# Janspiry/Image-Super-Resolution-via-Iterative-Refinement

Hardware: NVIDIA H100
Metric: diffusion steps/sec (batch16, 16->128 SR3) (higher is better)
Workload: dtype bf16

## Files before the change

### image-super-resolution-via-iterative-refinement_b200/_native.py

```python
import ctypes
import os
from ctypes import POINTER, c_char_p, c_double, c_float, c_int, c_int64, c_uint64, c_void_p

import torch

_PKG = os.path.dirname(os.path.abspath(__file__))
LIB_PATH = os.path.join(_PKG, "lib", "libsr3_b200.so")
SR3_MAX_LEVELS = 8
_lib = None


class NativeLibraryError(RuntimeError):
    pass


class UNetConfigC(ctypes.Structure):
    _fields_ = [("in_channel", c_int), ("out_channel", c_int), ("inner_channel", c_int), ("norm_groups", c_int),
                ("n_mults", c_int), ("channel_mults", c_int * SR3_MAX_LEVELS), ("n_attn_res", c_int),
                ("attn_res", c_int * SR3_MAX_LEVELS), ("res_blocks", c_int), ("image_size", c_int), ("channels", c_int),
                ("conditional", c_int), ("precision", c_int)]


PRECISIONS = {"bf16": 0, "fp32": 1}


class GemmGeometryC(ctypes.Structure):
    _fields_ = [(n, c_int) for n in ("tall", "mh", "block_n", "h_box", "b_box", "ksplit", "stages", "ctas", "tiles", "res_smem")]


class TestConvArgsC(ctypes.Structure):
    _fields_ = [("x", c_void_p), ("w", c_void_p), ("bias", c_void_p), ("bias2", c_void_p), ("resid", c_void_p),
                ("x2", c_void_p), ("w2", c_void_p),
                ("y", c_void_p), ("y_bf16", c_void_p), ("stats", c_void_p)] + \
               [(n, c_int) for n in ("B", "H", "W", "Cin", "Cout", "Cin2", "ksize", "stride", "fold_up", "precise")]


class TestGroupNormArgsC(ctypes.Structure):
    _fields_ = [(n, c_void_p) for n in ("x0", "x1", "st0", "st1", "gamma", "beta", "drop_mask", "dA", "add", "a_bf16", "mr", "dst0", "dst0_b",
                                         "gsum0", "dst1", "dgamma", "dbeta")] + \
               [("drop_seed", c_uint64)] + [(n, c_int) for n in ("B", "HW", "C0", "C1", "groups", "silu", "drop", "add_ld", "acc0")] + \
               [("drop_layer", ctypes.c_uint), ("drop_p", c_float), ("gscale", c_float)]


class TestFilmArgsC(ctypes.Structure):
    _fields_ = [(n, c_void_p) for n in ("wf", "tau", "dfilm", "nl", "w1", "b1", "w2", "dwf", "dbf", "dcb", "dtau", "dw1", "db1", "dw2", "db2")] + \
               [(n, c_int) for n in ("F", "inner", "B")] + [("gscale", c_float)]


_SIGS = {
    "sr3_last_error": (c_char_p, []),
    "sr3_abi_version": (c_int, []),
    "sr3_engine_create": (c_int, [POINTER(UNetConfigC), c_int, c_int, POINTER(c_void_p)]),
    "sr3_engine_create_sized": (c_int, [POINTER(UNetConfigC), c_int, c_int, c_int, c_int, POINTER(c_void_p)]),
    "sr3_engine_create_train": (c_int, [POINTER(UNetConfigC), c_int, c_int, c_float, POINTER(c_void_p)]),
    "sr3_train_forward": (c_int, [c_void_p, c_void_p, c_void_p, c_void_p, c_void_p, c_int, c_uint64, POINTER(c_double), c_void_p]),
    "sr3_train_backward": (c_int, [c_void_p, c_float, POINTER(c_void_p), c_int, c_void_p]),
    "sr3_train_num_backward_blocks": (c_int, [c_void_p]),
    "sr3_train_backward_begin": (c_int, [c_void_p, c_float, POINTER(c_void_p), c_int]),
    "sr3_train_backward_block": (c_int, [c_void_p, c_int, c_void_p]),
    "sr3_train_backward_flush": (c_int, [c_void_p, c_void_p]),
# ... 634 lines not shown
```

### image-super-resolution-via-iterative-refinement_b200/csrc/engine.cu

```cuda
#include <cuda.h>
#include <cuda_runtime.h>

#include <cmath>
#include <cstdarg>
#include <cstdlib>
#include <cstring>
#include <functional>
#include <limits>
#include <map>
#include <memory>
#include <mutex>
#include <stdexcept>
#include <string>
#include <vector>

#include "../../include/sr3_b200.h"
#include "aux_kernels.cuh"
#include "attn_wgmma.cuh"
#include "step_megakernel.cuh"
#include "train_kernels.cuh"

using namespace sr3;
typedef __nv_bfloat16 bf16;

// ... 362 lines not shown
        if (!d.out_f32) p.out_map = p.res_map;
        if (!d.resid) p.res_map = p.out_map;
        p.epi_c4_is_z = (d.out_f32 ? zo : zr) ? 1 : 0;
    } else {
        p.out_map = p.b_map; p.res_map = p.b_map;
    }
    p.ksplit = 1;
    {
        const int tiles = d.tiles_w * d.tiles_h * d.tiles_b * d.n_tiles * d.nz;
        const int ks = d.ksplit_max;
        if (ks > 1 && !d.pingpong && d.mode == 0 && d.out_f32 && d.block_n >= 32 && d.n_valid % 32 == 0) {
            int want = num_sms() / tiles;
            if (want > ks) want = ks;
            if (want > p.num_k * d.passes / 2) want = p.num_k * d.passes / 2;
            const int units = d.mh * (d.block_n / 32) * 4;
            if (want > units) want = units;
            want = fit_split(want, tiles);
            if (want > 1) {
                p.ksplit = want;
                p.ws = static_cast<float*>(mem.alloc((size_t)tiles * want * d.mh * 128 * d.block_n * sizeof(float), false));
                p.counters = static_cast<unsigned int*>(mem.alloc((size_t)tiles * sizeof(unsigned int)));
            }
        }
    }
    const int total_tiles = d.tiles_w * d.tiles_h * d.tiles_b * d.n_tiles * d.nz * p.ksplit;
    int ctas = total_tiles < num_sms() ? total_tiles : num_sms();
    if (const char* e = getenv("SR3_MAX_CTAS")) { int v = atoi(e); if (v > 0 && v < ctas) ctas = v; }
    REQUIRE(p.ksplit == 1 || ctas == total_tiles, "split-K launch needs one CTA per (tile, split) pair: %d CTAs for %d (SR3_MAX_CTAS with a split tile)", ctas, total_tiles);
    const dim3 grid(ctas, 1, 1);
    const int bn = d.block_n;
    const int mh = d.mh;
    const bool res_smem = p.tma_epi && d.resid != nullptr && p.ksplit <= 1;
    p.stages = pick_stages(d.block_n, p.a_stage_bytes, p.b_taps, res_smem, p.num_k);
    const int smem = gemm_smem_bytes(bn, p.a_stage_bytes, p.b_taps, p.stages, res_smem, p.num_k);
    REQUIRE(smem <= SMEM_LIMIT, "gemm shared memory %d exceeds the limit", smem);
    init_gemm_attrs();
    REQUIRE((bn == 16 || bn == 32 || bn == 64 || bn == 128 || bn == 256) && (mh == 1 || (mh == 2 && bn <= 128 && bn != 32)), "unsupported tile %dx%d", 128 * mh, bn);
    const bool pp = d.pingpong != 0;
    REQUIRE(!pp || (gemm_pingpong_ok(bn, mh) && p.ksplit == 1 && d.mode == 0), "no ping-pong form of tile %dx%d (split %d)", 128 * mh, bn, p.ksplit);
    if (geo) {
        geo->tall = d.tall; geo->mh = mh; geo->block_n = bn; geo->h_box = d.h_box; geo->b_box = d.b_box;
        geo->ksplit = p.ksplit; geo->stages = p.stages; geo->ctas = ctas; geo->tiles = total_tiles / p.ksplit; geo->res_smem = res_smem ? 1 : 0;
    }
    if (schedule) *schedule = pp ? 1 : 0;
    std::shared_ptr<GemmParams> sp = std::make_shared<GemmParams>(p);
    if (g_gemm_registry) {
        GemmHandle h; h.p = sp; h.w_ptr = d.b_ptr; h.w_bytes = 2LL * d.b_rows * d.b_K; h.w_is_param = d.b_is_param; h.bn = bn; h.mh = mh;
        g_gemm_registry->push_back(h);
    }
    if (g_mega_registry) {
        MegaRec r; r.type = MOP_GEMM; r.variant = bn | (mh << 16) | (pp ? MEGA_VARIANT_PP : 0); r.gp = sp;
        g_mega_registry->push_back(std::move(r));
    }
    return [sp, grid, bn, mh, pp, smem](cudaStream_t st) {
        const GemmParams& p = *sp;
        if (pp) {
            if (mh == 2) launch_gemm_bn<64, 2, true>(p, grid, smem, st);
            else if (bn == 64) launch_gemm_bn<64, 1, true>(p, grid, smem, st);
            else launch_gemm_bn<128, 1, true>(p, grid, smem, st);
            return;
        }
        switch (bn) {
            case 16: if (mh == 2) launch_gemm_bn<16, 2>(p, grid, smem, st); else launch_gemm_bn<16, 1>(p, grid, smem, st); break;
            case 32: launch_gemm_bn<32, 1>(p, grid, smem, st); break;
            case 64: if (mh == 2) launch_gemm_bn<64, 2>(p, grid, smem, st); else launch_gemm_bn<64, 1>(p, grid, smem, st); break;
            case 128: if (mh == 2) launch_gemm_bn<128, 2>(p, grid, smem, st); else launch_gemm_bn<128, 1>(p, grid, smem, st); break;
            default: launch_gemm_bn<256, 1>(p, grid, smem, st); break;
        }
    };
}

bool attn_fusable(int Lt, int C) { return (Lt == 128 || Lt == 256) && C % 128 == 0 && C >= 128; }

Op make_attn_op(const bf16* qk, const bf16* vT, bf16* out, int nz, int Lt, int HW, int C) {
    REQUIRE(attn_fusable(Lt, C) && Lt % HW == 0, "attention shape Lt=%d HW=%d C=%d is not supported by the fused kernel", Lt, HW, C);
// ... 698 lines not shown
    }
    void f32_param_into(const std::string& name, std::vector<int64_t> shape, float* dst) {
        if (dry) return;
        add_param(name, shape);
        PackDesc d{}; d.type = 0; d.dst = dst; d.n = params.back().numel; add_pack(name, d);
    }
    void conv_weight_param(const std::string& name, bf16* dst, int Cout, int Cin, int k, int ktot, int k_off, int cin_pad) {
        if (dry) return;
        add_param(name, {Cout, Cin, k, k});
        PackDesc d{}; d.type = 1; d.dst = dst; d.Cout = Cout; d.Cin = Cin; d.k = k; d.ld = PW * ktot; d.k_off = k_off; d.tap_stride = cin_pad;
        d.lo_off = precise ? ktot : 0;
        add_pack(name, d);
    }
    bf16* new_weight(int rows, int ktot) {
        if (dry) return nullptr;
        const int rows_pad = ((rows + 127) / 128) * 128;
        return static_cast<bf16*>(mem.alloc((size_t)rows_pad * PW * ktot * sizeof(bf16)));
    }
    void set_precise(GemmDesc& d, int c0, int c1, int ktot) {
        if (precise) set_precise_fields(d, c0, c1, ktot);
    }
    void push(Op op, int kind = 4, double flops = 0, double bytes = 0) {
        if (dry) return;
        if (bwd_sink) { bwd_sink->push_back(std::move(op)); bwd_kinds.back().push_back(kind); return; }
        ops.push_back(std::move(op));
        op_info.push_back({kind, flops, bytes, sr3_gemm_geometry{}, -1, {0, 0, 0}});
    }
    void push_gemm(const GemmDesc& d) {
        const double M = (double)d.OW * d.OH * d.OB * (d.nz > 1 && d.a_zstep == 0 ? d.nz : 1);
        const double K = 64.0 * d.slabs.size() * (d.passes > 1 ? d.passes : 1);
        const double N = d.n_valid;
        double bytes = N * K * 2;
        if (d.out_f32) bytes += M * N * 4;
        if (d.out_bf16) bytes += M * N * 2;
        if (d.resid) bytes += M * N * 4;
        double a_elems = 0;
        for (int i = 0; i < d.n_a; ++i) a_elems += (double)d.a[i].C * d.a[i].W * d.a[i].P * d.a[i].H * d.a[i].Bn;
        bytes += a_elems * 2;
        sr3_gemm_geometry geo{};
        int schedule = 0;
        push(make_gemm_op(d, mem, &geo, &schedule), 0, 2.0 * M * N * K, bytes);
        if (!dry && !bwd_sink) {
            OpInfo& info = op_info.back();
            info.geo = geo; info.schedule = schedule;
            info.out_hwc[0] = d.OH * (d.z_phase ? 2 : 1); info.out_hwc[1] = d.OW * (d.z_phase ? 2 : 1); info.out_hwc[2] = d.n_valid;
        }
    }

    float* last_mr = nullptr;
    void add_prep(const Act& s0, const Act* s1, const float* gamma, const float* beta, int groups, bool silu, bf16* out_a, bf16* out_raw, const DropSpec* drop = nullptr) {
        if (dry) return;
        PrepParams p = gn_op(s0.p, s0.stats, s0.C, s1 ? s1->p : nullptr, s1 ? s1->stats : nullptr, s1 ? s1->C : 0, gamma, beta, groups, s0.H * s0.W, silu);
        p.drop = drop;
        if (train) { last_mr = static_cast<float*>(mem.alloc((size_t)Bp * groups * 2 * sizeof(float))); p.save_mr = last_mr; }
        p.out_a = out_a; p.out_raw = out_raw; p.precise = precise ? 1 : 0;
        const int C = p.C0 + p.C1;
        const int vpp = C / 4;
        const RowLaunch L = prep_launch(C, groups, p.HW, B);
        p.pix_per_block = L.ppb;
        {
            PrepParams m = p;
            const int nth = GEMM_THREADS;
            const int kp = vpp > nth ? 1 : nth / vpp;
            int ipi = (4 * num_sms() + B / 2) / B; if (ipi < 1) ipi = 1;
            int mp = (p.HW + ipi - 1) / ipi;
            mp = ((mp + kp - 1) / kp) * kp;
            if (mp > p.HW) mp = p.HW;
// ... 1524 lines not shown
```

### image-super-resolution-via-iterative-refinement_b200/csrc/gemm_wgmma.cuh

```cuda
#pragma once
#include <cuda.h>
#include <type_traits>
#include "ptx.cuh"

namespace sr3 {

struct OutSpec {
    long long sZ, sB, sH, sW, off;
};

struct StepCtl {
    int t_cur;
    int t_next;
    int nl_from_table;
    int out_mode;
    int use_noise_buf;
    int write_mean;
    int clip;
    int update_state;
    unsigned long long seed;
    unsigned long long sample_offset;
};

struct PostParams {
// ... 8 lines not shown
    int in_C, in_coff;
    int in_lo_off;
};

struct StageTap {
    int a_chan;
    int dw, dh, p;
    int b_col;
    int a_off;
};
struct StageDesc {
    int ntaps;
    int a_multi;
    int a_sel;
    int pad0;
    StageTap tap[3];
    int pad1, pad2;
};

struct GemmParams {
    CUtensorMap a_map[2];
    CUtensorMap b_map;
    CUtensorMap out_map;
    CUtensorMap res_map;
    const StageDesc* ktab;
    int num_k;
    int a_stage_bytes;
    int a_box_bytes;
    int a_half_off;
    int b_taps;
    int tiles_w, tiles_h, tiles_b;
    int n_tiles, nz;
    int tma_epi;
    int epi_c4_is_z;
    int ksplit;
    float* ws;
    unsigned int* counters;
    const void* pf_ptr;
    long long pf_bytes;
    int w_box, h_box, b_box;
    int w_shift, h_shift;
    int a_zstep, b_zrows;
    int stages;
    int mode;
    int OW, OH, OB, n_valid;
    float scale;
    const float* bias;
    const float* bias2;
    int bias2_stride;
    const float* resid;
    OutSpec rs;
    float* out_f32;
    OutSpec os;
    __nv_bfloat16* out_bf16;
    OutSpec hs;
    __nv_bfloat16* out_t;
    int t_col0, t_rows, t_ld, t_per;
    double* stats;
    int stats_C, stats_coff;
    const StepCtl* ctl;
    PostParams post;
    int z_phase;
    long long z_off_hi, z_off_lo;
    int passes, lo_b_col, lo_a_chan[2];
    long long lo_out_off, lo_t_off;
    int t_fixed;
};

constexpr int GEMM_THREADS = 288;
constexpr int GEMM_EPI_WARPS = 8;
constexpr int GEMM_PRODUCER_WARP = 8;
constexpr int GEMM_MAX_STAGES = 8;
__host__ __device__ constexpr int gemm_epi_warp_bytes(bool resid) { return resid ? 12288 : 4096; }
__host__ __device__ constexpr int gemm_epi_bytes(bool resid) { return GEMM_EPI_WARPS * gemm_epi_warp_bytes(resid); }
constexpr int GEMM_MAX_K = 160;
constexpr int GEMM_HDR_BYTES = 2048;
constexpr int HDR_SCALARS = 512;
constexpr int HDR_PARAMS = 768;
constexpr int HDR_NUM_BARS = 64;
__host__ __device__ constexpr bool gemm_single_wg(int block_n, int mh) { return mh == 1 && block_n <= 32; }
__host__ __device__ constexpr bool gemm_pingpong_ok(int block_n, int mh) { return (mh == 2 && block_n == 64) || (mh == 1 && (block_n == 64 || block_n == 128)); }
constexpr int GEMM_ORDER_BAR = 2;
__host__ __device__ constexpr int gemm_stage_readers(int block_n, int mh, bool pp) { return (pp || gemm_single_wg(block_n, mh)) ? 1 : 2; }
__host__ __device__ constexpr int gemm_aux_bytes(int num_k) {
    return GEMM_HDR_BYTES + ((num_k * 96 + 127) / 128) * 128  + GEMM_EPI_WARPS * 2 * 32 * 4 ;
}

__host__ __device__ constexpr int gemm_stage_bytes(int block_n, int a_stage_bytes, int b_taps) { return a_stage_bytes + b_taps * block_n * 128; }
__host__ __device__ constexpr int gemm_smem_bytes(int block_n, int a_stage_bytes, int b_taps, int stages, bool resid, int num_k) {
    return stages * gemm_stage_bytes(block_n, a_stage_bytes, b_taps) + gemm_epi_bytes(resid) + 1024  + gemm_aux_bytes(num_k);
}

__device__ __forceinline__ void philox4x32_10(uint32_t (&c)[4], uint32_t k0, uint32_t k1) {
#pragma unroll
    for (int r = 0; r < 10; ++r) {
        const uint32_t hi0 = __umulhi(0xD2511F53u, c[0]), lo0 = 0xD2511F53u * c[0];
        const uint32_t hi1 = __umulhi(0xCD9E8D57u, c[2]), lo1 = 0xCD9E8D57u * c[2];
        const uint32_t n0 = hi1 ^ c[1] ^ k0, n1 = lo1, n2 = hi0 ^ c[3] ^ k1, n3 = lo0;
        c[0] = n0; c[1] = n1; c[2] = n2; c[3] = n3;
        k0 += 0x9E3779B9u; k1 += 0xBB67AE85u;
    }
}
__device__ __forceinline__ void box_muller(uint32_t a, uint32_t b, float& z0, float& z1) {
    const float u1 = (static_cast<float>(a) + 1.0f) * 2.3283064365386963e-10f;
    const float u2 = static_cast<float>(b) * 2.3283064365386963e-10f;
    const float r = sqrtf(-2.0f * logf(u1));
    float s, c;
    sincospif(2.0f * u2, &s, &c);
    z0 = r * c; z1 = r * s;
}

__device__ __forceinline__ double stats_quantize(double v) { return rint(v * 1048576.0) * (1.0 / 1048576.0); }

__device__ __forceinline__ float warp_column_sums(float (&v)[32]) {
    const uint32_t lane = lane_id();
#pragma unroll
    for (int half = 16; half >= 1; half >>= 1) {
        const bool up = (lane & half) != 0;
#pragma unroll
        for (int j = 0; j < half; ++j) {
            const float keep = up ? v[j + half] : v[j];
            const float send = up ? v[j] : v[j + half];
            v[j] = keep + __shfl_xor_sync(0xffffffffu, send, half);
// ... 26 lines not shown
        } else {
            uint32_t ctr[4] = {static_cast<uint32_t>(pix), static_cast<uint32_t>(ctl.sample_offset + img), static_cast<uint32_t>(t),
                               static_cast<uint32_t>((ctl.sample_offset + img) >> 32)};
            philox4x32_10(ctr, static_cast<uint32_t>(ctl.seed), static_cast<uint32_t>(ctl.seed >> 32));
            box_muller(ctr[0], ctr[1], z[0], z[1]);
            box_muller(ctr[2], ctr[3], z[2], z[3]);
        }
    }
    for (int c = 0; c < q.C; ++c) {
        const long long idx = (static_cast<long long>(img) * q.C + c) * plane + pix;
        const float xt = q.x_state[idx];
        float x0 = __fsub_rn(__fmul_rn(c1, xt), __fmul_rn(c2, eps[c]));
        if (ctl.clip) x0 = fminf(fmaxf(x0, -1.0f), 1.0f);
        const float mean = __fadd_rn(__fmul_rn(pc1, x0), __fmul_rn(pc2, xt));
        if (ctl.write_mean) q.mean_out[idx] = mean;
        const float xn = __fadd_rn(mean, __fmul_rn(z[c], sigma));
        if (ctl.update_state) {
            q.x_state[idx] = xn;
            __nv_bfloat16* ib = q.in_buf + (static_cast<long long>(img) * plane + pix) * q.in_C + q.in_coff + c;
            const __nv_bfloat16 hi = __float2bfloat16_rn(xn);
            *ib = hi;
            if (q.in_lo_off) ib[q.in_lo_off] = __float2bfloat16_rn(xn - __bfloat162float(hi));
        }
    }
}

static_assert(sizeof(GemmParams) <= GEMM_HDR_BYTES - HDR_PARAMS, "GemmParams must fit the shared-memory header");

__device__ __forceinline__ void gemm_stage_setup(const GemmParams& p, const GemmParams* pm, const uint32_t base, uint8_t* base_ptr, const int block_n,
                                                 const int mh, const bool pp, const bool recycle) {
    const int stages = p.stages;
    const int stage_bytes = p.a_stage_bytes + p.b_taps * block_n * 128;
    const bool use_res_tma = p.tma_epi && p.resid != nullptr && p.ksplit <= 1;
    const int epi_bytes = GEMM_EPI_WARPS * gemm_epi_warp_bytes(use_res_tma);
    uint8_t* aux_ptr = base_ptr + GEMM_HDR_BYTES + stages * stage_bytes + epi_bytes;
    {
        const int4* src = reinterpret_cast<const int4*>(p.ktab);
        int4* dst = reinterpret_cast<int4*>(aux_ptr);
        for (int i = threadIdx.x; i < p.num_k * 6; i += blockDim.x) dst[i] = __ldg(&src[i]);
    }
    if (threadIdx.x == 0) {
        tma_prefetch_desc(&pm->a_map[0]);
        tma_prefetch_desc(&pm->a_map[1]);
        tma_prefetch_desc(&pm->b_map);
        if (p.tma_epi) { tma_prefetch_desc(&pm->out_map); tma_prefetch_desc(&pm->res_map); }
        const uint32_t bar_base = base;
        if (recycle) {
            for (int i = 0; i < HDR_NUM_BARS; ++i) mbar_inval(bar_base + 8u * i);
        }
        const uint32_t consumers = gemm_stage_readers(block_n, mh, pp);
        for (int s = 0; s < stages; ++s) {
            mbar_init(bar_base + 8u * s, 1);
            mbar_init(bar_base + 8u * (GEMM_MAX_STAGES + s), consumers);
        }
        for (int w = 0; w < 2 * GEMM_EPI_WARPS; ++w) mbar_init(bar_base + 8u * (2 * GEMM_MAX_STAGES + w), 1);
        fence_mbar_init();
    }
}

template <int WN, int CW, int CL>
__device__ __forceinline__ void acc_chunk_rows(const float (&acc)[2][WN / 2], float* buf, float (&v)[32]) {
    static_assert(CW <= 32 && (CL + 1) * CW <= WN, "accumulator chunk");
    const int lane = static_cast<int>(lane_id());
    __syncwarp();
#pragma unroll
    for (int i = 0; i < 2; ++i) {
#pragma unroll
        for (int j = (CL * CW) / 2; j < ((CL + 1) * CW) / 2; j += 2) {
            const int r = (lane >> 2) + 8 * i + 16 * ((j >> 1) & 1);
            const int cc = 8 * (j >> 2) - CL * CW + 2 * (lane & 3);
            *reinterpret_cast<float2*>(buf + r * 32 + (cc ^ ((r & 7) << 2))) = make_float2(acc[i][j], acc[i][j + 1]);
        }
    }
    __syncwarp();
#pragma unroll
    for (int c4 = 0; c4 < CW / 4; ++c4) {
        const float4 x = *reinterpret_cast<const float4*>(buf + lane * 32 + ((4 * c4) ^ ((lane & 7) << 2)));
        v[4 * c4] = x.x; v[4 * c4 + 1] = x.y; v[4 * c4 + 2] = x.z; v[4 * c4 + 3] = x.w;
    }
}

template <int N, int I = 0, typename F>
__device__ __forceinline__ void static_for(F&& f) {
    if constexpr (I < N) {
        f(std::integral_constant<int, I>{});
        static_for<N, I + 1>(f);
    }
}
// ... 19 lines not shown
                }
            }
        }
        clear();
    }
    __device__ __forceinline__ void start(const GemmParams& p, const int im, const int nb0, const int ch0, const int lane) {
        if (im != img || nb0 != n0) { flush(p, ch0, lane); img = im; n0 = nb0; }
    }
    __device__ __forceinline__ void add(const int c, const double s, const double q) {
#pragma unroll
        for (int cc = 0; cc < N; ++cc)
            if (cc == c) { sum[cc] += s; sq[cc] += q; }
    }
};

template <int BLOCK_N, int MH, bool MEGA, bool PP = false>
__device__ __forceinline__ void gemm_tile_body(const GemmParams& p, const GemmParams* pm, const uint32_t base, uint8_t* base_ptr,
                                               const int cta, const int ncta) {
    static_assert(!PP || gemm_pingpong_ok(BLOCK_N, MH), "ping-pong tile shape");
    constexpr int B_BYTES = BLOCK_N * 128;
    constexpr bool SINGLE = !PP && gemm_single_wg(BLOCK_N, MH);
    constexpr int WN = (PP || SINGLE || MH == 2) ? BLOCK_N : BLOCK_N / 2;
    constexpr int AH = PP ? MH : 1;
    constexpr int CW = WN < 32 ? WN : 32;
    constexpr int NCH = BLOCK_N >= 32 ? BLOCK_N / 32 : 1;
    constexpr int NITEMS = MH * NCH;
    constexpr int OWN = PP ? NITEMS : SINGLE ? 1 : NITEMS / 2;
    constexpr int NSTAT = PP ? NCH : OWN;
    static_assert(WN % CW == 0 && AH * WN <= 128, "accumulator shape");

    const int stages = p.stages;
    const int stage_bytes = p.a_stage_bytes + p.b_taps * B_BYTES;
    const bool use_res_tma = p.tma_epi && p.resid != nullptr && p.ksplit <= 1;
    const int epi_warp_bytes = gemm_epi_warp_bytes(use_res_tma);
    const int epi_bytes = GEMM_EPI_WARPS * epi_warp_bytes;
    const uint32_t bar_base = base;
    const uint32_t stage_base = base + GEMM_HDR_BYTES;
    uint8_t* stage_ptr = base_ptr + GEMM_HDR_BYTES;
    const uint32_t epi_base = stage_base + stages * stage_bytes;
    auto full_bar = [&](int s) { return bar_base + 8u * s; };
    auto empty_bar = [&](int s) { return bar_base + 8u * (GEMM_MAX_STAGES + s); };
    auto res_bar = [&](int w, int b) { return bar_base + 8u * (2 * GEMM_MAX_STAGES + 2 * w + b); };
    uint8_t* aux_ptr = stage_ptr + stages * stage_bytes + epi_bytes;
    StageDesc* ktab_s = reinterpret_cast<StageDesc*>(aux_ptr);
    float* bias_s = reinterpret_cast<float*>(aux_ptr + ((p.num_k * 96 + 127) / 128) * 128);

    const int warp = threadIdx.x >> 5;
    const int lane = threadIdx.x & 31;
    const int tiles_m = p.tiles_w * p.tiles_h * p.tiles_b;
    const int ksplit = p.ksplit > 1 ? p.ksplit : 1;
    const int total_tiles = tiles_m * p.n_tiles * p.nz * ksplit;
    const int num_kt = p.num_k * (p.passes > 1 ? p.passes : 1);
    if constexpr (!MEGA) {
        gemm_stage_setup(p, pm, base, base_ptr, BLOCK_N, MH, PP, false);
        __syncthreads();
    }
    if (warp == 2 && lane == 0 && p.pf_bytes > 0) {
        long long chunk = ((p.pf_bytes + ncta - 1) / ncta + 15) & ~15ll;
        const long long off = chunk * cta;
        if (off < p.pf_bytes) {
            if (off + chunk > p.pf_bytes) chunk = (p.pf_bytes - off) & ~15ll;
            const char* src = static_cast<const char*>(p.pf_ptr) + off;
            for (long long done = 0; done < chunk; done += 65536) {
                const unsigned int n = static_cast<unsigned int>(chunk - done < 65536 ? chunk - done : 65536);
                if (n >= 16) asm volatile("cp.async.bulk.prefetch.L2.global [%0], %1;" ::"l"(src + done), "r"(n) : "memory");
            }
        }
    }
    if constexpr (!MEGA) {
        pdl_launch_dependents();
        pdl_wait();
    }

    auto decode = [&](int tile_s, int& w0, int& h0, int& b0, int& n0, int& z) {
        const int tile = tile_s / ksplit;
// ... 29 lines not shown
                    const int na = e.a_multi ? e.ntaps : 1;
                    mbar_arrive_expect_tx(full_bar(s), na * p.a_box_bytes + e.ntaps * B_BYTES);
                    for (int t = 0; t < na; ++t)
                        tma_load_5d(a_dst + (e.a_multi ? e.tap[t].a_off : 0), &pm->a_map[e.a_sel], full_bar(s), e.tap[t].a_chan + a_lo, w0 + e.tap[t].dw + zdw, e.tap[t].p,
                                    h0 + e.tap[t].dh + (e.a_multi ? zdh : 0), b0);
                    for (int t = 0; t < e.ntaps; ++t)
                        tma_load_2d(a_dst + p.a_stage_bytes + t * B_BYTES, &pm->b_map, full_bar(s), e.tap[t].b_col + b_lo, brow);
                }
                __syncwarp();
                if (++s == stages) { s = 0; ph ^= 1u; }
            }
        }
        if constexpr (MEGA) {
            int filled = 0;
            for (int tile = tile_begin; tile < tile_end; ++tile) {
                const int sp = tile % ksplit;
                filled += (num_kt * (sp + 1)) / ksplit - (num_kt * sp) / ksplit;
            }
            const int n_wait = filled < stages ? filled : stages;
            for (int i = 0; i < n_wait; ++i) {
                mbar_wait(empty_bar(s), ph ^ 1u);
                if (++s == stages) { s = 0; ph ^= 1u; }
            }
        }
    } else if (warp < GEMM_EPI_WARPS) {
        const int g = warp >> 2;
        const int q = warp & 3;
        const int ew = warp;
        const bool mma_wg = !SINGLE || g == 0;
        const int own0 = (SINGLE || PP) ? 0 : g * OWN;
        const int ch0 = PP ? 0 : own0 % NCH;
        const int acc_half = (MH == 2 && !PP) ? g : 0;
        const int acc_c0 = (MH == 1 && !SINGLE && !PP) ? g * WN : 0;
        const uint32_t out_smem = epi_base + ew * epi_warp_bytes;
        const uint32_t res_smem = out_smem + 4096;
        uint8_t* out_ptr = stage_ptr + stages * stage_bytes + ew * epi_warp_bytes;
        uint8_t* res_ptr = out_ptr + 4096;
        const bool use_out_tma = p.tma_epi && p.out_f32 != nullptr;
        uint32_t res_phase = 0;
        uint32_t res_count = 0;
        uint32_t bias_slot = 0;
        bool out_pending = false;
        int s = 0;
        uint32_t ph = 0;
        StatRun<NSTAT> st_own;
        for (int tile = tile_begin + (PP ? g : 0); tile < tile_end; tile += (PP ? 2 : 1)) {
            float acc[AH][2][WN / 2];
            int w0, h0, b0, n0, z;
            decode(tile, w0, h0, b0, n0, z);
            if constexpr (PP) {
                const long long pos = static_cast<long long>(tile - tile_begin) * num_kt;
                s = static_cast<int>(pos % stages);
                ph = static_cast<uint32_t>((pos / stages) & 1);
            }
            auto item_geom = [&](int item, int qq, int& half, int& ch, int& sw, int& sh, int& c4) {
                half = item / NCH; ch = item % NCH;
                const int r0 = half * 128 + qq * 32;
                sw = r0 & (p.w_box - 1);
                sh = (r0 >> p.w_shift) & (p.h_box - 1);
                const int sb = r0 >> (p.w_shift + p.h_shift);
                c4 = p.epi_c4_is_z ? z : (b0 + sb);
            };
            auto request_resid = [&](int item) {
                int half, ch, sw, sh, c4;
                item_geom(item, q, half, ch, sw, sh, c4);
                const uint32_t b = res_count & 1;
                mbar_arrive_expect_tx(res_bar(ew, b), 4096);
                tma_load_5d(res_smem + b * 4096, &pm->res_map, res_bar(ew, b), n0 + ch * 32, w0 + sw, 0, h0 + sh, c4);
            };
            auto item_bias = [&](int item, int qq) {
                float bv = 0.f;
                const int half = item / NCH, ch = item % NCH;
                const int img = b0 + ((half * 128 + qq * 32) >> (p.w_shift + p.h_shift));
                const int n = n0 + ch * 32 + lane;
                if (n < p.n_valid) {
                    if (p.bias) bv += __ldg(&p.bias[n]);
                    if (p.bias2) bv += __ldcg(&p.bias2[static_cast<long long>(img < p.OB ? img : 0) * p.bias2_stride + n]);
                }
                return bv;
            };
            constexpr int WJ = MH * 128;
            auto ws_row = [&](int item, int qq) {
                return (static_cast<long long>(item % NCH) * 8 * WJ + (item / NCH) * 128 + qq * 32 + lane) * 4;
            };
            if (use_res_tma && mma_wg && lane == 0) request_resid(own0);
            float bvs[OWN] = {};
            if constexpr (BLOCK_N != 16) {
                if (mma_wg) {
#pragma unroll
                    for (int ii = 0; ii < OWN; ++ii) bvs[ii] = item_bias(own0 + ii, q);
                }
            }
            const int sp = tile % ksplit;
            if (mma_wg) {
                const int k0 = (num_kt * sp) / ksplit, k1 = (num_kt * (sp + 1)) / ksplit;
                int zrow_off = 0;
                if (p.z_phase) {
                    const int zz = (tile / ksplit) / (tiles_m * p.n_tiles);
                    zrow_off = (zz >> 1) * 1024;
                }
                const uint32_t a_base = stage_base + acc_half * p.a_half_off;
                const uint32_t b_base = stage_base + p.a_stage_bytes + acc_c0 * 128;
                const int li = tile - tile_begin;
                if (PP && li > 0) asm volatile("bar.sync %0, 256;" ::"r"(GEMM_ORDER_BAR + g) : "memory");
                int prev = -1;
                for (int k = k0; k < k1; ++k) {
                    mbar_wait(full_bar(s), ph);
                    const StageDesc& e = ktab_s[k % p.num_k];
                    const int ntaps = __shfl_sync(0xffffffffu, e.ntaps, 0);
                    auto issue = [&](auto nt_c) {
                        wgmma_fence();
#pragma unroll
                        for (int t = 0; t < decltype(nt_c)::value; ++t) {
                            const uint32_t a_addr = a_base + s * stage_bytes + e.tap[t].a_off + (e.a_multi ? 0 : zrow_off);
                            const uint32_t b_addr = b_base + s * stage_bytes + t * B_BYTES;
#pragma unroll
                            for (int kk = 0; kk < 4; ++kk) {
                                const uint64_t bdesc = wgmma_desc_sw128(b_addr + kk * 32, 16, 1024);
// ... 30 lines not shown
                    wgmma_fence_regs(acc[hh][0]);
                    wgmma_fence_regs(acc[hh][1]);
                }
                if (prev >= 0) mbar_arrive_if(empty_bar(prev), (threadIdx.x & 127) == 0);
            }
            const int npass = (!PP && ksplit > 1) ? 2 : 1;
            constexpr long long SLICE = static_cast<long long>(MH) * 128 * BLOCK_N;
#pragma unroll 1
            for (int pass = 0; pass < npass; ++pass) {
            if (pass == 1) {
                __threadfence();
                asm volatile("bar.sync 1, 256;" ::: "memory");
                if (ew == 0 && lane == 0) {
                    unsigned int* ctr = p.counters + tile / ksplit;
                    const unsigned int old = atomicAdd(ctr, 1u);
                    const unsigned int target = (old / ksplit + 1u) * ksplit;
                    uint64_t t0 = 0;
                    for (uint32_t spins = 0;; ++spins) {
                        unsigned int v;
                        asm volatile("ld.acquire.gpu.global.u32 %0, [%1];" : "=r"(v) : "l"(ctr) : "memory");
                        if (static_cast<int>(v - target) >= 0) break;
                        if ((spins & 1023u) == 1023u) {
                            const uint64_t now = globaltimer_ns();
                            if (t0 == 0) t0 = now;
                            if (now - t0 > 4000000000ull) __trap();
                        }
                    }
                    __threadfence();
                }
                __syncwarp();
                asm volatile("bar.sync 1, 256;" ::: "memory");
            }
            const bool to_ws = (!PP && ksplit > 1 && pass == 0);
            auto epi_item = [&](const int item, const int qq, const float bv, const bool last, auto&& fetch, auto&& add_stats) {
                int half, ch, sw, sh, c4;
                item_geom(item, qq, half, ch, sw, sh, c4);
                const int row = half * 128 + qq * 32 + lane;
                const int w = row & (p.w_box - 1);
                const int h = (row >> p.w_shift) & (p.h_box - 1);
                const int bb = row >> (p.w_shift + p.h_shift);
                const int ow = w0 + w, oh = h0 + h, img = b0 + bb;
                const bool row_ok = (ow < p.OW) && (oh < p.OH) && (img < p.OB);
                float v[32];
                if constexpr (BLOCK_N == 16) {
                    fetch(v);
                    if (row_ok) {
                        float eps[4] = {0.f, 0.f, 0.f, 0.f};
                        for (int c = 0; c < p.post.C; ++c) eps[c] = v[c] + __ldg(&p.bias[c]);
                        final_epilogue(p, eps, img, oh, ow);
                    }
                } else {
                    const int nb = n0 + ch * 32;
                    float* bs = bias_s + (ew * 2 + (bias_slot++ & 1u)) * 32;
                    bs[lane] = bv;
                    __syncwarp();
                    if (use_res_tma) {
                        ++res_count;
                        if (!last && lane == 0) request_resid(item + 1);
                    }
                    fetch(v);
                    const float ep_scale = p.scale;
                    const bool full = (nb + 32 <= p.n_valid);
#pragma unroll
                    for (int j4 = 0; j4 < 8; ++j4) {
                        const float4 bq = reinterpret_cast<const float4*>(bs)[j4];
                        const float bb4[4] = {bq.x, bq.y, bq.z, bq.w};
#pragma unroll
                        for (int jj = 0; jj < 4; ++jj) {
                            const int j = 4 * j4 + jj;
                            float x = v[j] * ep_scale + bb4[jj];
                            if (!full && nb + j >= p.n_valid) x = 0.f;
                            v[j] = x;
                        }
                    }
                    if (use_res_tma) {
                        const uint32_t b = (res_count - 1) & 1;
                        mbar_wait(res_bar(ew, b), (res_phase >> b) & 1u);
                        res_phase ^= (1u << b);
                        const uint8_t* rp = res_ptr + b * 4096 + lane * 128;
#pragma unroll
                        for (int j = 0; j < 8; ++j) {
                            const float4 r = *reinterpret_cast<const float4*>(rp + ((j ^ (lane & 7)) << 4));
                            v[4 * j] += r.x; v[4 * j + 1] += r.y; v[4 * j + 2] += r.z; v[4 * j + 3] += r.w;
                        }
                        __syncwarp();
                    } else if (row_ok && p.resid) {
                        const long long ro = out_index(p.rs, z, img, oh, ow);
                        for (int j = 0; j < 32; ++j)
                            if (nb + j < p.n_valid) v[j] += __ldcg(&p.resid[ro + nb + j]);
                    }
                    if (use_out_tma) {
                        if (out_pending) {
                            if (lane == 0) tma_store_wait_read<0>();
                            __syncwarp();
                        }
                        uint8_t* op = out_ptr + lane * 128;
#pragma unroll
                        for (int j = 0; j < 8; ++j)
                            *reinterpret_cast<float4*>(op + ((j ^ (lane & 7)) << 4)) = make_float4(v[4 * j], v[4 * j + 1], v[4 * j + 2], v[4 * j + 3]);
                        fence_proxy_async_smem();
                        __syncwarp();
                        if (lane == 0) {
                            if (p.z_phase) tma_store_5d(&pm->out_map, out_smem, (z & 1) * p.n_valid + nb, w0 + sw, z >> 1, h0 + sh, c4);
                            else tma_store_5d(&pm->out_map, out_smem, nb, w0 + sw, 0, h0 + sh, c4);
                            tma_store_commit();
                        }
                        out_pending = true;
                    } else if (row_ok && p.out_f32) {
                        const long long oo = out_index(p.os, z, img, oh, ow) + (p.z_phase ? (z >> 1) * p.z_off_hi + (z & 1) * p.z_off_lo : 0);
                        if (full) {
                            float4* o4 = reinterpret_cast<float4*>(p.out_f32 + oo + nb);
#pragma unroll
                            for (int j = 0; j < 8; ++j) o4[j] = make_float4(v[4 * j], v[4 * j + 1], v[4 * j + 2], v[4 * j + 3]);
                        } else {
                            for (int j = 0; j < 32; ++j)
                                if (nb + j < p.n_valid) p.out_f32[oo + nb + j] = v[j];
                        }
                    }
                    if (p.out_t && nb >= p.t_col0) {
                        if (ow < p.OW && oh < p.OH && nb + 32 <= p.n_valid) {
                            __nv_bfloat16* tp = p.out_t + (static_cast<long long>(img / p.t_per) * p.t_rows + (nb - p.t_col0)) * p.t_ld +
                                                (img % p.t_per) * (p.OH * p.OW) + oh * p.OW + ow;
#pragma unroll
                            for (int j = 0; j < 32; ++j) {
                                const __nv_bfloat16 hi = __float2bfloat16_rn(v[j]);
                                tp[static_cast<long long>(j) * p.t_ld] = hi;
                                if (p.lo_t_off) tp[static_cast<long long>(j) * p.t_ld + p.lo_t_off] = __float2bfloat16_rn(v[j] - __bfloat162float(hi));
                            }
// ... 53 lines not shown
                                    const float x0 = *reinterpret_cast<const float*>(colp + r * 128 + ((cq4 ^ (r & 7)) << 4)) - sft;
                                    const float x1 = *reinterpret_cast<const float*>(colp + (r + 1) * 128 + ((cq4 ^ ((r + 1) & 7)) << 4)) - sft;
                                    a0 += x0; q0 = fmaf(x0, x0, q0);
                                    a1 += x1; q1 = fmaf(x1, x1, q1);
                                }
                            } else {
#pragma unroll
                                for (int r = 0; r < 32; r += 2) {
                                    float x0 = *reinterpret_cast<const float*>(colp + r * 128 + ((cq4 ^ (r & 7)) << 4)) - sft;
                                    float x1 = *reinterpret_cast<const float*>(colp + (r + 1) * 128 + ((cq4 ^ ((r + 1) & 7)) << 4)) - sft;
                                    if (!((okm >> r) & 1u)) x0 = 0.f;
                                    if (!((okm >> (r + 1)) & 1u)) x1 = 0.f;
                                    a0 += x0; q0 = fmaf(x0, x0, q0);
                                    a1 += x1; q1 = fmaf(x1, x1, q1);
                                }
                            }
                            const double n_ok = static_cast<double>(__popc(okm)), ds = static_cast<double>(sft);
                            const double da = static_cast<double>(a0 + a1), dq = static_cast<double>(q0 + q1);
                            cs = da + n_ok * ds;
                            cq = dq + 2.0 * ds * da + n_ok * ds * ds;
                        } else {
                            float s2[32];
#pragma unroll
                            for (int j = 0; j < 32; ++j) {
                                const float x = row_ok ? v[j] : 0.f;
                                v[j] = x; s2[j] = x * x;
                            }
                            cs = static_cast<double>(warp_column_sums(v));
                            cq = static_cast<double>(warp_column_sums(s2));
                        }
                        add_stats(cs, cq);
                    }
                }
            };
            if (pass == 0) {
                if (mma_wg) {
                    if (!PP && p.stats && !to_ws) st_own.start(p, b0 + ((acc_half * 128 + q * 32) >> (p.w_shift + p.h_shift)), n0, ch0, lane);
                    static_for<OWN>([&](auto ii_c) {
                        constexpr int ii = decltype(ii_c)::value;
                        constexpr int AHI = PP ? ii / NCH : 0, ACL = PP ? ii % NCH : ii;
                        if constexpr (PP) {
                            if (ACL == 0 && p.stats) st_own.start(p, b0 + ((AHI * 128 + q * 32) >> (p.w_shift + p.h_shift)), n0, 0, lane);
                        }
                        auto stage_acc = [&](float (&v)[32]) {
                            if (out_pending) {
                                if (lane == 0) tma_store_wait_read<0>();
                                __syncwarp();
                            }
                            acc_chunk_rows<WN, CW, ACL>(acc[AHI], reinterpret_cast<float*>(out_ptr), v);
                        };
                        if (to_ws) {
                            float v[32];
                            stage_acc(v);
                            float4* dst = reinterpret_cast<float4*>(p.ws + static_cast<long long>(tile) * SLICE + ws_row(own0 + ii, q));
#pragma unroll
                            for (int j = 0; j < 8; ++j) __stcg(dst + j * WJ, make_float4(v[4 * j], v[4 * j + 1], v[4 * j + 2], v[4 * j + 3]));
                        } else {
                            epi_item(own0 + ii, q, bvs[ii], ii + 1 == OWN, stage_acc, [&](double cs, double cq) { st_own.add(PP ? ACL : ii, cs, cq); });
                        }
                    });
                }
            } else {
                StatRun<NCH> st_ws;
#pragma unroll 1
                for (int it = sp + ksplit * ew; it < NITEMS * 4; it += ksplit * GEMM_EPI_WARPS) {
                    const int item = it >> 2, qq = it & 3;
                    if (p.stats) st_ws.start(p, b0 + (((item / NCH) * 128 + qq * 32) >> (p.w_shift + p.h_shift)), n0, 0, lane);
                    epi_item(item, qq, BLOCK_N != 16 ? item_bias(item, qq) : 0.f, true,
                             [&](float (&v)[32]) {
                                 const float* src0 = p.ws + static_cast<long long>(tile - sp) * SLICE + ws_row(item, qq);
#pragma unroll
                                 for (int j = 0; j < 32; ++j) v[j] = 0.f;
                                 for (int s2 = 0; s2 < ksplit; ++s2) {
                                     const float4* src = reinterpret_cast<const float4*>(src0 + s2 * SLICE);
#pragma unroll
                                     for (int j = 0; j < 8; ++j) {
                                         const float4 r = __ldcg(src + j * WJ);
                                         v[4 * j] += r.x; v[4 * j + 1] += r.y; v[4 * j + 2] += r.z; v[4 * j + 3] += r.w;
                                     }
                                 }
                             },
                             [&](double cs, double cq) { st_ws.add(item % NCH, cs, cq); });
                }
                if (p.stats) st_ws.flush(p, 0, lane);
            }
            }
        }
        if (p.stats) st_own.flush(p, ch0, lane);
        if constexpr (MEGA) {
            if (use_out_tma && out_pending && lane == 0) tma_store_wait_all<0>();
        } else {
            if (use_out_tma && out_pending && lane == 0) tma_store_wait_read<0>();
        }
    }
}

template <int BLOCK_N, int MH, bool PP = false>
__global__ void __launch_bounds__(GEMM_THREADS, 1) gemm_tile_kernel(const __grid_constant__ GemmParams p) {
    extern __shared__ uint8_t smem_raw[];
    const uint32_t raw = smem_u32(smem_raw);
    const uint32_t base = (raw + 1023u) & ~1023u;
// ... 5 lines not shown
```

### include/sr3_b200.h

```cpp
#ifndef SR3_B200_H
#define SR3_B200_H

#include <stdint.h>

#ifdef __cplusplus
extern "C" {
#endif

#define SR3_MAX_LEVELS 8

typedef struct sr3_unet_config {
    int in_channel;
    int out_channel;
    int inner_channel;
    int norm_groups;
    int n_mults;
    int channel_mults[SR3_MAX_LEVELS];
    int n_attn_res;
    int attn_res[SR3_MAX_LEVELS];
    int res_blocks;
    int image_size;
    int channels;
    int conditional;
    int precision;
// ... 51 lines not shown
                              uint64_t first_sample_index, float* final_host, void* stream);

int sr3_p_sample_loop_begin(sr3_engine* e, const float* condition_x, const float* x_T, uint64_t seed, uint64_t first_sample_index, void* stream);
int sr3_p_sample_steps(sr3_engine* e, int t_start, int steps, void* stream);
int sr3_read_state(sr3_engine* e, float* x_out, void* stream);

int sr3_tensor2img(const float* src, unsigned char* dst_u8, int n, int C, int H, int W, int nrow, float min_v, float max_v, void* stream);
int sr3_ssd_u8(const unsigned char* a_u8, const unsigned char* b_u8, int64_t n, unsigned long long* ssd_host, void* stream);
int sr3_ssim(const void* a, const void* b, int dtype, int n, int H, int W, int C, double* ssim_host, void* stream);
int sr3_image_metrics(const float* sr_f32, const float* hr_f32, int n, int C, int H, int W, float min_v, float max_v, unsigned char* sr_u8,
                      unsigned char* hr_u8, unsigned long long* ssd_host, double* ssim_host, void* stream);

int sr3_pil_bicubic_tables(int in_size, int out_size, int* bounds, int* coef, int coef_cap, int* ksize);
int sr3_resize_bicubic_u8(const unsigned char* src_u8, unsigned char* dst_u8, float* dst_f32, int B, int h, int w, int C, int H, int W, int flip,
                          float min_v, float max_v, void* stream);

int sr3_engine_num_launches_per_step(const sr3_engine* e);
int sr3_engine_num_ops_per_step(const sr3_engine* e);
int sr3_engine_uses_step_kernel(const sr3_engine* e);
int sr3_engine_step_kernel_profile(sr3_engine* e, int cap, int* types, double* us, double* phases_or_null, int* n_ops, void* stream);
int64_t sr3_engine_workspace_bytes(const sr3_engine* e);
int sr3_engine_profile_step(sr3_engine* e, int t, int reps, int cap, int* kinds, float* ms, double* flops, double* bytes, int* n_ops,
                            void* stream);
int sr3_engine_read_activation(sr3_engine* e, const char* name, float* dst, int64_t cap, int64_t* numel, int shape_bhwc[4], void* stream);

int sr3_test_gemm(const void* a_bf16, const void* b_bf16, float* d, int M, int N, int K, int block_n, void* stream);
int sr3_test_attention(const void* qk_bf16, const void* vT_bf16, void* out_bf16, int nz, int Lt, int HW, int C, void* stream);
int sr3_test_attention_unfused(const void* qk_bf16, const void* vT_bf16, float* S, void* P_bf16, void* O_bf16, int nz, int Lt, int HW, int C,
                               int precise, void* stream);
int sr3_test_conv(const void* x_bf16, const float* w_oihw, const float* bias, float* y, double* stats, int B, int H, int W, int Cin,
                  int Cout, int ksize, int stride, void* stream);

typedef struct sr3_gemm_geometry {
    int tall, mh, block_n, h_box, b_box, ksplit, stages, ctas, tiles, res_smem;
} sr3_gemm_geometry;
typedef struct sr3_test_conv_args {
    const void* x; const float* w; const float* bias; const float* bias2; const float* resid;
    const void* x2; const float* w2;
    float* y; void* y_bf16; double* stats;
    int B, H, W, Cin, Cout, Cin2, ksize, stride;
    int fold_up, precise;
} sr3_test_conv_args;
int sr3_test_conv_ex(const sr3_test_conv_args* args, sr3_gemm_geometry* geometry, void* stream);
int sr3_tile_schedule(const sr3_engine* e, int op, sr3_gemm_geometry* geometry, int* schedule, int* out_hwc);
int sr3_test_wgrad(const void* dy_bf16, const void* x_bf16, float* grad, int B, int OH, int OW, int CY, int Cin, int ksize, int stride,
                   int cout_valid, int cin_valid, int slices, float gscale, int raw, int* slices_used, void* stream);

int sr3_test_conv_groupnorm(const void* x_bf16, const float* w_oihw, const float* bias, const float* gamma, const float* beta, int groups,
                            int silu, float* y, void* a_bf16, int B, int H, int W, int Cin, int Cout, int ksize, void* stream);


typedef struct sr3_test_groupnorm_args {
    const float* x0; const float* x1; const double* st0; const double* st1; const float* gamma; const float* beta;
    const unsigned char* drop_mask; const float* dA; const float* add;
    void* a_bf16; float* mr; float* dst0; void* dst0_b; float* gsum0; float* dst1; float* dgamma; float* dbeta;
    uint64_t drop_seed;
    int B, HW, C0, C1, groups, silu, drop, add_ld, acc0;
    unsigned int drop_layer;
    float drop_p, gscale;
} sr3_test_groupnorm_args;
int sr3_test_groupnorm_layer(const sr3_test_groupnorm_args* args, void* stream);
int sr3_test_grad_combine(const float* a, const float* b, float* dst, int acc, void* dst_b, float* gsum, float* bias0, float* bias1, float gscale,
                          int B, int HW, int C, void* stream);
int sr3_test_dgrad(const void* dy_bf16, const float* w_oihw, float* dx, int form, int B, int H, int W, int CY, int Cin, int Cout, int ksize,
                   void* stream);
int sr3_test_attention_bwd(const void* qk_bf16, const void* vT_bf16, const void* P_bf16, const void* dO_bf16, float* dS, void* dS_bf16, float* dqkv,
                           void* dqkv_bf16, int nz, int Lt, int HW, int C, void* stream);
// ... 19 lines not shown
```

Measured before the change: 140.5.

## Double-buffer GEMM epilogue output staging and prefetch residuals across tiles

Adds a second per-warp shared-memory slot for the TMA output store when it fits in shared memory, so the epilogue waits only for the older store rather than all outstanding stores. Residual TMA loads are now issued from a global request counter that runs ahead across tile boundaries instead of restarting per tile, which keeps the residual prefetch pipeline full. Both aim to hide epilogue store and load latency, at the cost of more shared memory per CTA and a more complex barrier-phase scheme. The byte accounting for profiling was also updated for the dual bf16 output.

```diff
diff --git a/image-super-resolution-via-iterative-refinement_b200/_native.py b/image-super-resolution-via-iterative-refinement_b200/_native.py
--- a/image-super-resolution-via-iterative-refinement_b200/_native.py
+++ b/image-super-resolution-via-iterative-refinement_b200/_native.py
@@ -25,7 +25,8 @@
 
 
 class GemmGeometryC(ctypes.Structure):
-    _fields_ = [(n, c_int) for n in ("tall", "mh", "block_n", "h_box", "b_box", "ksplit", "stages", "ctas", "tiles", "res_smem")]
+    _fields_ = [(n, c_int) for n in ("tall", "mh", "block_n", "h_box", "b_box", "ksplit", "stages", "ctas", "tiles", "res_smem",
+                                                 "epi_slots")]
 
 
 class TestConvArgsC(ctypes.Structure):
diff --git a/image-super-resolution-via-iterative-refinement_b200/csrc/engine.cu b/image-super-resolution-via-iterative-refinement_b200/csrc/engine.cu
--- a/image-super-resolution-via-iterative-refinement_b200/csrc/engine.cu
+++ b/image-super-resolution-via-iterative-refinement_b200/csrc/engine.cu
@@ -418,7 +418,11 @@
     const int mh = d.mh;
     const bool res_smem = p.tma_epi && d.resid != nullptr && p.ksplit <= 1;
     p.stages = pick_stages(d.block_n, p.a_stage_bytes, p.b_taps, res_smem, p.num_k);
-    const int smem = gemm_smem_bytes(bn, p.a_stage_bytes, p.b_taps, p.stages, res_smem, p.num_k);
+    p.epi_slots = 1;
+    while (p.tma_epi && d.out_f32 && p.epi_slots < GEMM_EPI_MAX_SLOTS &&
+           gemm_smem_bytes(bn, p.a_stage_bytes, p.b_taps, p.stages, res_smem, p.num_k, p.epi_slots + 1) <= SMEM_LIMIT)
+        ++p.epi_slots;
+    const int smem = gemm_smem_bytes(bn, p.a_stage_bytes, p.b_taps, p.stages, res_smem, p.num_k, p.epi_slots);
     REQUIRE(smem <= SMEM_LIMIT, "gemm shared memory %d exceeds the limit", smem);
     init_gemm_attrs();
     REQUIRE((bn == 16 || bn == 32 || bn == 64 || bn == 128 || bn == 256) && (mh == 1 || (mh == 2 && bn <= 128 && bn != 32)), "unsupported tile %dx%d", 128 * mh, bn);
@@ -427,6 +431,7 @@
     if (geo) {
         geo->tall = d.tall; geo->mh = mh; geo->block_n = bn; geo->h_box = d.h_box; geo->b_box = d.b_box;
         geo->ksplit = p.ksplit; geo->stages = p.stages; geo->ctas = ctas; geo->tiles = total_tiles / p.ksplit; geo->res_smem = res_smem ? 1 : 0;
+        geo->epi_slots = p.epi_slots;
     }
     if (schedule) *schedule = pp ? 1 : 0;
     std::shared_ptr<GemmParams> sp = std::make_shared<GemmParams>(p);
@@ -1191,7 +1196,7 @@
         const double N = d.n_valid;
         double bytes = N * K * 2;
         if (d.out_f32) bytes += M * N * 4;
-        if (d.out_bf16) bytes += M * N * 2;
+        if (d.out_bf16) bytes += M * N * 2 * (d.lo_out_off ? 2 : 1);
         if (d.resid) bytes += M * N * 4;
         double a_elems = 0;
         for (int i = 0; i < d.n_a; ++i) a_elems += (double)d.a[i].C * d.a[i].W * d.a[i].P * d.a[i].H * d.a[i].Bn;
diff --git a/image-super-resolution-via-iterative-refinement_b200/csrc/gemm_wgmma.cuh b/image-super-resolution-via-iterative-refinement_b200/csrc/gemm_wgmma.cuh
--- a/image-super-resolution-via-iterative-refinement_b200/csrc/gemm_wgmma.cuh
+++ b/image-super-resolution-via-iterative-refinement_b200/csrc/gemm_wgmma.cuh
@@ -64,6 +64,7 @@
     int tiles_w, tiles_h, tiles_b;
     int n_tiles, nz;
     int tma_epi;
+    int epi_slots;
     int epi_c4_is_z;
     int ksplit;
     float* ws;
@@ -103,8 +104,10 @@
 constexpr int GEMM_EPI_WARPS = 8;
 constexpr int GEMM_PRODUCER_WARP = 8;
 constexpr int GEMM_MAX_STAGES = 8;
-__host__ __device__ constexpr int gemm_epi_warp_bytes(bool resid) { return resid ? 12288 : 4096; }
-__host__ __device__ constexpr int gemm_epi_bytes(bool resid) { return GEMM_EPI_WARPS * gemm_epi_warp_bytes(resid); }
+constexpr int GEMM_EPI_MAX_SLOTS = 2;
+constexpr int GEMM_RES_SLOTS = 2;
+__host__ __device__ constexpr int gemm_epi_warp_bytes(bool resid, int slots = 1) { return slots * 4096 + (resid ? GEMM_RES_SLOTS * 4096 : 0); }
+__host__ __device__ constexpr int gemm_epi_bytes(bool resid, int slots = 1) { return GEMM_EPI_WARPS * gemm_epi_warp_bytes(resid, slots); }
 constexpr int GEMM_MAX_K = 160;
 constexpr int GEMM_HDR_BYTES = 2048;
 constexpr int HDR_SCALARS = 512;
@@ -119,8 +122,8 @@
 }
 
 __host__ __device__ constexpr int gemm_stage_bytes(int block_n, int a_stage_bytes, int b_taps) { return a_stage_bytes + b_taps * block_n * 128; }
-__host__ __device__ constexpr int gemm_smem_bytes(int block_n, int a_stage_bytes, int b_taps, int stages, bool resid, int num_k) {
-    return stages * gemm_stage_bytes(block_n, a_stage_bytes, b_taps) + gemm_epi_bytes(resid) + 1024  + gemm_aux_bytes(num_k);
+__host__ __device__ constexpr int gemm_smem_bytes(int block_n, int a_stage_bytes, int b_taps, int stages, bool resid, int num_k, int epi_slots = 1) {
+    return stages * gemm_stage_bytes(block_n, a_stage_bytes, b_taps) + gemm_epi_bytes(resid, epi_slots) + 1024  + gemm_aux_bytes(num_k);
 }
 
 __device__ __forceinline__ void philox4x32_10(uint32_t (&c)[4], uint32_t k0, uint32_t k1) {
@@ -213,7 +216,7 @@
     const int stages = p.stages;
     const int stage_bytes = p.a_stage_bytes + p.b_taps * block_n * 128;
     const bool use_res_tma = p.tma_epi && p.resid != nullptr && p.ksplit <= 1;
-    const int epi_bytes = GEMM_EPI_WARPS * gemm_epi_warp_bytes(use_res_tma);
+    const int epi_bytes = gemm_epi_bytes(use_res_tma, p.epi_slots);
     uint8_t* aux_ptr = base_ptr + GEMM_HDR_BYTES + stages * stage_bytes + epi_bytes;
     {
         const int4* src = reinterpret_cast<const int4*>(p.ktab);
@@ -234,7 +237,7 @@
             mbar_init(bar_base + 8u * s, 1);
             mbar_init(bar_base + 8u * (GEMM_MAX_STAGES + s), consumers);
         }
-        for (int w = 0; w < 2 * GEMM_EPI_WARPS; ++w) mbar_init(bar_base + 8u * (2 * GEMM_MAX_STAGES + w), 1);
+        for (int w = 0; w < GEMM_RES_SLOTS * GEMM_EPI_WARPS; ++w) mbar_init(bar_base + 8u * (2 * GEMM_MAX_STAGES + w), 1);
         fence_mbar_init();
     }
 }
@@ -320,7 +323,8 @@
     const int stages = p.stages;
     const int stage_bytes = p.a_stage_bytes + p.b_taps * B_BYTES;
     const bool use_res_tma = p.tma_epi && p.resid != nullptr && p.ksplit <= 1;
-    const int epi_warp_bytes = gemm_epi_warp_bytes(use_res_tma);
+    const int epi_slots = p.epi_slots;
+    const int epi_warp_bytes = gemm_epi_warp_bytes(use_res_tma, epi_slots);
     const int epi_bytes = GEMM_EPI_WARPS * epi_warp_bytes;
     const uint32_t bar_base = base;
     const uint32_t stage_base = base + GEMM_HDR_BYTES;
@@ -328,7 +332,8 @@
     const uint32_t epi_base = stage_base + stages * stage_bytes;
     auto full_bar = [&](int s) { return bar_base + 8u * s; };
     auto empty_bar = [&](int s) { return bar_base + 8u * (GEMM_MAX_STAGES + s); };
-    auto res_bar = [&](int w, int b) { return bar_base + 8u * (2 * GEMM_MAX_STAGES + 2 * w + b); };
+    auto res_bar = [&](int w, int b) { return bar_base + 8u * (2 * GEMM_MAX_STAGES + GEMM_RES_SLOTS * w + b); };
+    static_assert(2 * GEMM_MAX_STAGES + GEMM_RES_SLOTS * GEMM_EPI_WARPS <= HDR_NUM_BARS, "mbarriers");
     uint8_t* aux_ptr = stage_ptr + stages * stage_bytes + epi_bytes;
     StageDesc* ktab_s = reinterpret_cast<StageDesc*>(aux_ptr);
     float* bias_s = reinterpret_cast<float*>(aux_ptr + ((p.num_k * 96 + 127) / 128) * 128);
@@ -424,17 +429,50 @@
         const int ch0 = PP ? 0 : own0 % NCH;
         const int acc_half = (MH == 2 && !PP) ? g : 0;
         const int acc_c0 = (MH == 1 && !SINGLE && !PP) ? g * WN : 0;
-        const uint32_t out_smem = epi_base + ew * epi_warp_bytes;
-        const uint32_t res_smem = out_smem + 4096;
-        uint8_t* out_ptr = stage_ptr + stages * stage_bytes + ew * epi_warp_bytes;
-        uint8_t* res_ptr = out_ptr + 4096;
+        const uint32_t out_smem0 = epi_base + ew * epi_warp_bytes;
+        const uint32_t res_smem = out_smem0 + epi_slots * 4096;
+        uint8_t* out_ptr0 = stage_ptr + stages * stage_bytes + ew * epi_warp_bytes;
+        uint8_t* res_ptr = out_ptr0 + epi_slots * 4096;
         const bool use_out_tma = p.tma_epi && p.out_f32 != nullptr;
-        uint32_t res_phase = 0;
-        uint32_t res_count = 0;
+        int out_slot = 0;
         uint32_t bias_slot = 0;
         bool out_pending = false;
         int s = 0;
         uint32_t ph = 0;
+        auto wait_slot = [&]() {
+            static_assert(GEMM_EPI_MAX_SLOTS == 2, "wait depths");
+            if (out_pending) {
+                if (lane == 0) {
+                    if (epi_slots > 1) tma_store_wait_read<1>();
+                    else tma_store_wait_read<0>();
+                }
+                __syncwarp();
+            }
+        };
+        auto item_geom = [&](int item, int qq, int b0, int z, int& half, int& ch, int& sw, int& sh, int& c4) {
+            half = item / NCH; ch = item % NCH;
+            const int r0 = half * 128 + qq * 32;
+            sw = r0 & (p.w_box - 1);
+            sh = (r0 >> p.w_shift) & (p.h_box - 1);
+            const int sb = r0 >> (p.w_shift + p.h_shift);
+            c4 = p.epi_c4_is_z ? z : (b0 + sb);
+        };
+        const int my_tile0 = tile_begin + (PP ? g : 0), my_step = PP ? 2 : 1;
+        const int res_total = (use_res_tma && mma_wg && my_tile0 < tile_end) ? ((tile_end - my_tile0 + my_step - 1) / my_step) * OWN : 0;
+        int res_req = 0;
+        int res_count = 0;
+        auto request_resid = [&]() {
+            int w0, h0, b0, n0, z;
+            decode(my_tile0 + (res_req / OWN) * my_step, w0, h0, b0, n0, z);
+            int half, ch, sw, sh, c4;
+            item_geom(own0 + res_req % OWN, q, b0, z, half, ch, sw, sh, c4);
+            const int b = res_req % GEMM_RES_SLOTS;
+            mbar_arrive_expect_tx(res_bar(ew, b), 4096);
+            tma_load_5d(res_smem + b * 4096, &pm->res_map, res_bar(ew, b), n0 + ch * 32, w0 + sw, 0, h0 + sh, c4);
+            ++res_req;
+        };
+        if (lane == 0)
+            while (res_req < res_total && res_req < GEMM_RES_SLOTS) request_resid();
         StatRun<NSTAT> st_own;
         for (int tile = tile_begin + (PP ? g : 0); tile < tile_end; tile += (PP ? 2 : 1)) {
             float acc[AH][2][WN / 2];
@@ -445,21 +483,6 @@
                 s = static_cast<int>(pos % stages);
                 ph = static_cast<uint32_t>((pos / stages) & 1);
             }
-            auto item_geom = [&](int item, int qq, int& half, int& ch, int& sw, int& sh, int& c4) {
-                half = item / NCH; ch = item % NCH;
-                const int r0 = half * 128 + qq * 32;
-                sw = r0 & (p.w_box - 1);
-                sh = (r0 >> p.w_shift) & (p.h_box - 1);
-                const int sb = r0 >> (p.w_shift + p.h_shift);
-                c4 = p.epi_c4_is_z ? z : (b0 + sb);
-            };
-            auto request_resid = [&](int item) {
-                int half, ch, sw, sh, c4;
-                item_geom(item, q, half, ch, sw, sh, c4);
-                const uint32_t b = res_count & 1;
-                mbar_arrive_expect_tx(res_bar(ew, b), 4096);
-                tma_load_5d(res_smem + b * 4096, &pm->res_map, res_bar(ew, b), n0 + ch * 32, w0 + sw, 0, h0 + sh, c4);
-            };
             auto item_bias = [&](int item, int qq) {
                 float bv = 0.f;
                 const int half = item / NCH, ch = item % NCH;
@@ -475,7 +498,6 @@
             auto ws_row = [&](int item, int qq) {
                 return (static_cast<long long>(item % NCH) * 8 * WJ + (item / NCH) * 128 + qq * 32 + lane) * 4;
             };
-            if (use_res_tma && mma_wg && lane == 0) request_resid(own0);
             float bvs[OWN] = {};
             if constexpr (BLOCK_N != 16) {
                 if (mma_wg) {
@@ -572,9 +594,9 @@
                 asm volatile("bar.sync 1, 256;" ::: "memory");
             }
             const bool to_ws = (!PP && ksplit > 1 && pass == 0);
-            auto epi_item = [&](const int item, const int qq, const float bv, const bool last, auto&& fetch, auto&& add_stats) {
+            auto epi_item = [&](const int item, const int qq, const float bv, auto&& fetch, auto&& add_stats) {
                 int half, ch, sw, sh, c4;
-                item_geom(item, qq, half, ch, sw, sh, c4);
+                item_geom(item, qq, b0, z, half, ch, sw, sh, c4);
                 const int row = half * 128 + qq * 32 + lane;
                 const int w = row & (p.w_box - 1);
                 const int h = (row >> p.w_shift) & (p.h_box - 1);
@@ -591,13 +613,11 @@
                     }
                 } else {
                     const int nb = n0 + ch * 32;
-                    float* bs = bias_s + (ew * 2 + (bias_slot++ & 1u)) * 32;
+                    uint8_t* const out_ptr = out_ptr0 + out_slot * 4096;
+                    const uint32_t out_smem = out_smem0 + out_slot * 4096;
+                    float* bs =bias_s + (ew * 2 + (bias_slot++ & 1u)) * 32;
                     bs[lane] = bv;
                     __syncwarp();
-                    if (use_res_tma) {
-                        ++res_count;
-                        if (!last && lane == 0) request_resid(item + 1);
-                    }
                     fetch(v);
                     const float ep_scale = p.scale;
                     const bool full = (nb + 32 <= p.n_valid);
@@ -614,9 +634,8 @@
                         }
                     }
                     if (use_res_tma) {
-                        const uint32_t b = (res_count - 1) & 1;
-                        mbar_wait(res_bar(ew, b), (res_phase >> b) & 1u);
-                        res_phase ^= (1u << b);
+                        const int b = res_count % GEMM_RES_SLOTS;
+                        mbar_wait(res_bar(ew, b), static_cast<uint32_t>(res_count / GEMM_RES_SLOTS) & 1u);
                         const uint8_t* rp = res_ptr + b * 4096 + lane * 128;
 #pragma unroll
                         for (int j = 0; j < 8; ++j) {
@@ -624,16 +643,15 @@
                             v[4 * j] += r.x; v[4 * j + 1] += r.y; v[4 * j + 2] += r.z; v[4 * j + 3] += r.w;
                         }
                         __syncwarp();
+                        ++res_count;
+                        if (lane == 0 && res_req < res_total) request_resid();
                     } else if (row_ok && p.resid) {
                         const long long ro = out_index(p.rs, z, img, oh, ow);
                         for (int j = 0; j < 32; ++j)
                             if (nb + j < p.n_valid) v[j] += __ldcg(&p.resid[ro + nb + j]);
                     }
                     if (use_out_tma) {
-                        if (out_pending) {
-                            if (lane == 0) tma_store_wait_read<0>();
-                            __syncwarp();
-                        }
+                        wait_slot();
                         uint8_t* op = out_ptr + lane * 128;
 #pragma unroll
                         for (int j = 0; j < 8; ++j)
@@ -753,6 +771,7 @@
                         add_stats(cs, cq);
                     }
                 }
+                if (++out_slot == epi_slots) out_slot = 0;
             };
             if (pass == 0) {
                 if (mma_wg) {
@@ -764,11 +783,8 @@
                             if (ACL == 0 && p.stats) st_own.start(p, b0 + ((AHI * 128 + q * 32) >> (p.w_shift + p.h_shift)), n0, 0, lane);
                         }
                         auto stage_acc = [&](float (&v)[32]) {
-                            if (out_pending) {
-                                if (lane == 0) tma_store_wait_read<0>();
-                                __syncwarp();
-                            }
-                            acc_chunk_rows<WN, CW, ACL>(acc[AHI], reinterpret_cast<float*>(out_ptr), v);
+                            wait_slot();
+                            acc_chunk_rows<WN, CW, ACL>(acc[AHI], reinterpret_cast<float*>(out_ptr0 + out_slot * 4096), v);
                         };
                         if (to_ws) {
                             float v[32];
@@ -777,7 +793,7 @@
 #pragma unroll
                             for (int j = 0; j < 8; ++j) __stcg(dst + j * WJ, make_float4(v[4 * j], v[4 * j + 1], v[4 * j + 2], v[4 * j + 3]));
                         } else {
-                            epi_item(own0 + ii, q, bvs[ii], ii + 1 == OWN, stage_acc, [&](double cs, double cq) { st_own.add(PP ? ACL : ii, cs, cq); });
+                            epi_item(own0 + ii, q, bvs[ii], stage_acc, [&](double cs, double cq) { st_own.add(PP ? ACL : ii, cs, cq); });
                         }
                     });
                 }
@@ -787,7 +803,7 @@
                 for (int it = sp + ksplit * ew; it < NITEMS * 4; it += ksplit * GEMM_EPI_WARPS) {
                     const int item = it >> 2, qq = it & 3;
                     if (p.stats) st_ws.start(p, b0 + (((item / NCH) * 128 + qq * 32) >> (p.w_shift + p.h_shift)), n0, 0, lane);
-                    epi_item(item, qq, BLOCK_N != 16 ? item_bias(item, qq) : 0.f, true,
+                    epi_item(item, qq, BLOCK_N != 16 ? item_bias(item, qq) : 0.f,
                              [&](float (&v)[32]) {
                                  const float* src0 = p.ws + static_cast<long long>(tile - sp) * SLICE + ws_row(item, qq);
 #pragma unroll
diff --git a/include/sr3_b200.h b/include/sr3_b200.h
--- a/include/sr3_b200.h
+++ b/include/sr3_b200.h
@@ -107,7 +107,7 @@
                   int Cout, int ksize, int stride, void* stream);
 
 typedef struct sr3_gemm_geometry {
-    int tall, mh, block_n, h_box, b_box, ksplit, stages, ctas, tiles, res_smem;
+    int tall, mh, block_n, h_box, b_box, ksplit, stages, ctas, tiles, res_smem, epi_slots;
 } sr3_gemm_geometry;
 typedef struct sr3_test_conv_args {
     const void* x; const float* w; const float* bias; const float* bias2; const float* resid;
```

Result: no change. 141.9, median of 6 (+1.0%).
